# FlagArihant2000/sfm-mvs

Hardware: AMD Instinct MI355X
Metric: descriptor-pair distances/sec (BF-KNN k=2 + Lowe ratio) (higher is better)
Workload: dtype f32 results (bit-identical to the direct-form f32 reference); filter arithmetic on MFMA: i8 MFMA on the descriptors QUANTISED to 8 bits (one grid per pair; the certificate uses the measured residua...; 1 GPU; BASELINE configs[1]: 10k x 10k uniform[0,1) float32 128-D descriptors, BF-KNN k=2 + Lowe ratio 0.70; a step = one launch set = a batch of 8 distinct pairs of that shape per GPU (8e8 distances; 8 distinct pairs per launch set, 2 sets of images rotating over the steps); nq=10000, nt=10000, dim=128

## Files before the change

### sfm_mvs_amd/csrc/knn.hip

```cpp
#include "common.h"
#include <cfloat>
#include <climits>
#include <cstdlib>
#include <type_traits>
#include <algorithm>
#include <mutex>
#include <vector>

namespace {

typedef float f32x16 __attribute__((ext_vector_type(16)));
typedef float f32x4 __attribute__((ext_vector_type(4)));
typedef float f32x3 __attribute__((ext_vector_type(3), aligned(4)));
typedef int i32x3 __attribute__((ext_vector_type(3), aligned(4)));

constexpr int kDim = 128;
constexpr int kTileT = 32;


constexpr int kResidentWaves = 4096;
constexpr int kMaxSlots = 258;
constexpr float kInf = __builtin_huge_valf();
constexpr int kSubTilesHost = 64;
constexpr int kI8SubTilesHost = 128;
// ... 399 lines not shown
                    const unsigned ad = (abase ^ (32u * ((c + 2) & 7))) + ((c + 2) >= 8 ? 256u : 0u);
                    asm volatile("ds_read_b128 %0, %1" : "=v"(af[(c + 2) % 3]) : "v"(ad));
                    asm volatile("s_waitcnt lgkmcnt(2)" : "+v"(af[c % 3]));
                } else if (c + 1 < 16) {
                    asm volatile("s_waitcnt lgkmcnt(1)" : "+v"(af[c % 3]));
                } else {
                    asm volatile("s_waitcnt lgkmcnt(0)" : "+v"(af[c % 3]));
                }
                __builtin_amdgcn_sched_barrier(0);
                acc = __builtin_amdgcn_mfma_f32_32x32x2f32(af[c % 3][0], bq[4 * c + 0], acc, 0, 0, 0);
                acc = __builtin_amdgcn_mfma_f32_32x32x2f32(af[c % 3][1], bq[4 * c + 1], acc, 0, 0, 0);
                acc = __builtin_amdgcn_mfma_f32_32x32x2f32(af[c % 3][2], bq[4 * c + 2], acc, 0, 0, 0);
                acc = __builtin_amdgcn_mfma_f32_32x32x2f32(af[c % 3][3], bq[4 * c + 3], acc, 0, 0, 0);
            }
            acc = __builtin_amdgcn_mfma_f32_32x32x2f32(aug_a, aug_b, acc, 0, 0, 0);
            if (ABL & 16) __builtin_amdgcn_s_setprio(0);
            const int seq0 = (t - sub_t0) << 2;
            if (ABL & 1) {
                k0 = min(k0, __float_as_int(acc[0]) + __float_as_int(acc[15]));
            } else
#pragma unroll
            for (int r = 0; r < 16; r += 4) {
                const int key = (min(min(__float_as_int(acc[r]), __float_as_int(acc[r + 1])), min(__float_as_int(acc[r + 2]), __float_as_int(acc[r + 3]))) & ~kKeyMask) | (seq0 + (r >> 2));
                const int lo = min(key, k0), hi = max(key, k0);
                const int m1 = max(min(key, k1), min(max(key, k1), k0));
                k2 = max(min(key, k1), min(max(key, k1), k2));
                k1 = m1;
                k0 = lo;
                (void)hi;
            }
            if (!(ABL & 2)) __syncthreads();
        }

        if (qok) {
            flush_keys(k0, k1, k2, sub_t0, h, cand_s + obase + 6 * sub, cand_i + obase + 6 * sub);
            for (int e = sub + 1; e < nsub; ++e)
#pragma unroll
                for (int r = 0; r < 3; ++r) {
                    cand_s[obase + 6 * e + r] = kInf;
                    cand_i[obase + 6 * e + r] = -1;
                }
        }
        u += t_end - t_begin;
    }
    if (trace && threadIdx.x == 0) trace[4 * blockIdx.x + 1] = wall_clock64();
}

typedef __bf16 bf16x8 __attribute__((ext_vector_type(8)));
typedef _Float16 f16x8 __attribute__((ext_vector_type(8)));
typedef unsigned u32x4 __attribute__((ext_vector_type(4)));
typedef _Float16 f16x2 __attribute__((ext_vector_type(2)));
typedef float f32x2 __attribute__((ext_vector_type(2)));

__device__ __forceinline__ float dot8_f16(const uint4& a, const uint4& b, float c) {
    c = __builtin_amdgcn_fdot2(__builtin_bit_cast(f16x2, a.x), __builtin_bit_cast(f16x2, b.x), c, false);
    c = __builtin_amdgcn_fdot2(__builtin_bit_cast(f16x2, a.y), __builtin_bit_cast(f16x2, b.y), c, false);
    c = __builtin_amdgcn_fdot2(__builtin_bit_cast(f16x2, a.z), __builtin_bit_cast(f16x2, b.z), c, false);
    c = __builtin_amdgcn_fdot2(__builtin_bit_cast(f16x2, a.w), __builtin_bit_cast(f16x2, b.w), c, false);
    return c;
}

__device__ __forceinline__ unsigned bf16_rn_bits(float x) {
    const unsigned u = __float_as_uint(x);
    return (u + 0x7FFFu + ((u >> 16) & 1u)) >> 16;
}

constexpr int kModeHalfExact = 0, kModeHalf = 1, kModeSplit = 2;
constexpr int kFlagHalfInexact = 2, kFlagRangeBad = 4, kFlagNotU8 = 8, kFlagSomeU8 = 16;
constexpr int kFlagQ8 = 32;

template <int M>
__device__ __forceinline__ int lane_xor(int v) {
    if constexpr (M == 1) return __builtin_amdgcn_update_dpp(0, v, 0xB1 , 0xF, 0xF, false);
    else if constexpr (M == 2) return __builtin_amdgcn_update_dpp(0, v, 0x4E , 0xF, 0xF, false);
    else if constexpr (M == 4 || M == 8 || M == 16) return __builtin_amdgcn_ds_swizzle(v, 0x1F | (M << 10));
    else return __shfl_xor(v, M, 64);
}
template <int M>
__device__ __forceinline__ float lane_xor(float v) { return __int_as_float(lane_xor<M>(__float_as_int(v))); }
__device__ __forceinline__ int knn_filter_mode(const int* __restrict__ flags, const float* __restrict__ bmax, int lane,
                                               float* tmax_out = nullptr) {
    const int fl = flags[lane] | flags[lane + 64] | flags[lane + 128] | flags[lane + 192];
    float tmax = fmaxf(fmaxf(bmax[lane], bmax[lane + 64]), fmaxf(bmax[lane + 128], bmax[lane + 192]));
#pragma unroll
    for (int m = 32; m >= 1; m >>= 1) tmax = fmaxf(tmax, __shfl_xor(tmax, m, 64));
    if (tmax_out) *tmax_out = tmax;
    if (__any((fl & kFlagRangeBad) != 0)) return kModeSplit;
    if (!__any((fl & kFlagHalfInexact) != 0)) return kModeHalfExact;
    return tmax >= 0.25f ? kModeHalf : kModeSplit;
}

constexpr int kMinfoPairMode = 0, kMinfoBatchMode = kMaxBatch, kMinfoTmax = 16, kMinfoTerr = 24, kMinfoQmax = 32, kMinfoBase = 40, kMinfoI8 = 48,
              kMinfoQ8 = 49,
              kMinfoSub8 = 50,
              kMinfoTicket = 51,
              kMinfoQ8S = 56, kMinfoQ8Lo = 64,
              kMinfoWords = 72;
__device__ __forceinline__ int knn_batch_mode(const int* __restrict__ flags, const float* __restrict__ bmax, int n_pairs, int lane) {
    int mode = kModeHalfExact;
    for (int b = 0; b < n_pairs; ++b) mode = max(mode, knn_filter_mode(flags + b * kNormBlocks, bmax + b * kNormBlocks, lane));
    return mode;
}

constexpr int kFragBytes = 1024;
constexpr int kInitFragBytes = 512;
constexpr int kTileFragBytes = 8 * kFragBytes + kInitFragBytes;

__device__ __forceinline__ uint2 frag_init_operand(float x, bool query_side, int h) {
    unsigned hi = bf16_rn_bits(x), mid = 0, lo = 0;
    if (x < kInf) {
        const float r1 = x - __uint_as_float(hi << 16);
        mid = bf16_rn_bits(r1);
        lo = bf16_rn_bits(r1 - __uint_as_float(mid << 16));
    }
    const unsigned one = 0x3F80u;
    if (query_side) return h == 0 ? make_uint2(one | (one << 16), one | (hi << 16)) : make_uint2(mid | (lo << 16), 0u);
    return h == 0 ? make_uint2(hi | (mid << 16), lo | (one << 16)) : make_uint2(one | (one << 16), 0u);
}

constexpr int kI8Groups = 8;
constexpr int kI8Rows = 4 * kI8Groups * 32;
constexpr int kI8SubTiles = 128;
constexpr int kI8TileBytes = 5 * 1024;
constexpr int kI8QTileBytes = 4 * 1024;
constexpr int kI8CMax = 508031, kI8CMin = -503936;
static_assert(kI8SubTiles == kI8SubTilesHost, "make_plan's copy");
constexpr int kKeyEmptyI = 0x7FFFFF00;

constexpr int kQ8SubTiles = 32;
static_assert(kQ8SubTiles == kQ8SubTilesHost, "make_plan's copy");
struct Q8Grid {
    float lo, s, inv;
    int kind;
};
__device__ __forceinline__ Q8Grid q8_sample_grid(const float* __restrict__ Q, int64_t ldq, int nq, const float* __restrict__ T, int64_t ldt, int nt,
                                                 float* __restrict__ red ) {
    const int sr = threadIdx.x >> 4, c = threadIdx.x & 15;
    const float* qs = Q + (int64_t)(((int64_t)sr * nq) >> 4) * ldq + 8 * c;
    const float* ts = T + (int64_t)(((int64_t)sr * nt) >> 4) * ldt + 8 * c;
    const float4 v0 = *reinterpret_cast<const float4*>(qs), v1 = *reinterpret_cast<const float4*>(qs + 4);
    const float4 v2 = *reinterpret_cast<const float4*>(ts), v3 = *reinterpret_cast<const float4*>(ts + 4);
    const float in[16] = {v0.x, v0.y, v0.z, v0.w, v1.x, v1.y, v1.z, v1.w, v2.x, v2.y, v2.z, v2.w, v3.x, v3.y, v3.z, v3.w};
    float mn = kInf, mx = -kInf, sm = 0.f, sq = 0.f;
    bool bad = false, nonu8 = false;
#pragma unroll
    for (int e = 0; e < 16; ++e) {
        mn = fminf(mn, in[e]);
        mx = fmaxf(mx, in[e]);
        sm += in[e];
        sq = fmaf(in[e], in[e], sq);
        bad = bad || !(fabsf(in[e]) < kInf);
        nonu8 = nonu8 || !(in[e] >= 0.f && in[e] <= 255.f && in[e] == floorf(in[e]));
    }
#pragma unroll
    for (int m = 32; m >= 1; m >>= 1) {
        mn = fminf(mn, __shfl_xor(mn, m, 64));
        mx = fmaxf(mx, __shfl_xor(mx, m, 64));
        sm += __shfl_xor(sm, m, 64);
        sq += __shfl_xor(sq, m, 64);
    }
    const int fl = (__any(bad) ? 1 : 0) | (__any(nonu8) ? 2 : 0);
    __syncthreads();
    if ((threadIdx.x & 63) == 0) {
        red[5 * (threadIdx.x >> 6)] = mn;
        red[5 * (threadIdx.x >> 6) + 1] = mx;
        red[5 * (threadIdx.x >> 6) + 2] = __int_as_float(fl);
        red[5 * (threadIdx.x >> 6) + 3] = sm;
        red[5 * (threadIdx.x >> 6) + 4] = sq;
    }
    __syncthreads();
    int flw = 0;
    mn = red[0]; mx = red[1]; sm = 0.f; sq = 0.f;
#pragma unroll
    for (int w = 0; w < 4; ++w) {
        mn = fminf(mn, red[5 * w]);
        mx = fmaxf(mx, red[5 * w + 1]);
        flw |= __float_as_int(red[5 * w + 2]);
        sm += red[5 * w + 3];
        sq += red[5 * w + 4];
    }
    Q8Grid g{0.f, 1.f, 1.f, 0};
    if (flw & 1) { g.kind = 2; return g; }
    if (!(flw & 2)) return g;
    const float s = (mx - mn) * (1.f / 255.f), mabs = fmaxf(fabsf(mn), fabsf(mx));
    if (!(s >= 1e-12f && s <= 1e30f && s >= 1.52587890625e-05f * mabs)) { g.kind = 2; return g; }
    {
        const float mean = sm * (1.f / 4096.f), var = fmaxf(sq * (1.f / 4096.f) - mean * mean, 0.f);
        if (!((mx - mn) * (mx - mn) <= 25.f * var)) { g.kind = 2; return g; }
    }
    g.lo = mn; g.s = s; g.inv = 1.f / s; g.kind = 1;
    return g;
}

__device__ __forceinline__ float fp16_chunk(const float (&in)[8], float sc, unsigned (&fw)[4], unsigned& flags) {
    fw[0] = fw[1] = fw[2] = fw[3] = 0u;
    float err2 = 0.f;
    unsigned amax = 0u, umin = 0xFFFFFFFFu, dor = 0u;
#pragma unroll
    for (int e = 0; e < 8; ++e) {
        const float ev = sc * in[e];
        const _Float16 hv = (_Float16)ev;
        fw[e >> 1] |= (unsigned)__builtin_bit_cast(unsigned short, hv) << (16 * (e & 1));
        const float dv = ev - (float)hv;
        err2 = fmaf(dv, dv, err2);
        const unsigned ab = __float_as_uint(ev) & 0x7FFFFFFFu;
        amax = max(amax, ab);
        umin = min(umin, ab - 1u);
        dor |= __float_as_uint(dv);
    }
    if (amax > 0x476A6000u ) flags |= kFlagRangeBad;
    const bool has_sub = umin < 0x38800000u - 1u;
    if ((dor & 0x7FFFFFFFu) != 0u || has_sub) flags |= kFlagHalfInexact;
    if (has_sub) {
        err2 = 0.f;
#pragma unroll
        for (int e = 0; e < 8; ++e) {
            const float ev = sc * in[e];
            const float dv = fabsf(ev) < 6.103515625e-5f ? ev : ev - (float)__builtin_bit_cast(_Float16, (unsigned short)(fw[e >> 1] >> (16 * (e & 1))));
            err2 = fmaf(dv, dv, err2);
        }
    }
    return err2;
}

constexpr int kPrepThreads = 256;
__global__ __launch_bounds__(kPrepThreads) void knn_prep_kernel(BatchPtrs P, int64_t ldq, int nq, int nq_pad,
                                                       int64_t ldt, int nt, int nt_pad,
                                                       unsigned short* __restrict__ qsplit, float* __restrict__ qn,
                                                       unsigned short* __restrict__ tsplit, float* __restrict__ tn,
                                                       float* __restrict__ bmax, int* __restrict__ midflag,
                                                       float* __restrict__ qerr , float* __restrict__ bmaxerr ,
                                                       float* __restrict__ bqmax ,
                                                       int64_t s_qsplit, int64_t s_tsplit, int64_t s_qn, int64_t s_tn,
                                                       unsigned char* __restrict__ qfrag ,
                                                       unsigned char* __restrict__ tfrag, int64_t s_qfrag, int64_t s_tfrag,
                                                       int* __restrict__ zero, int nzero,
                                                       int64_t units, int tiles, int G, int seg_cost, int n_rb,
                                                       int64_t* __restrict__ wg_begin, int* __restrict__ rb_first,
                                                       int* __restrict__ rb_last, int* __restrict__ wg_sbase,
                                                       unsigned char* __restrict__ qi8, unsigned char* __restrict__ ti8, int64_t s_qi8, int64_t s_ti8,
                                                       int* __restrict__ wq , int* __restrict__ wt ,
                                                       int* __restrict__ bwmin , int* __restrict__ bwmax,
                                                       unsigned short* __restrict__ rmq ,
                                                       unsigned short* __restrict__ rmt ,
                                                       int64_t units8, int G8, int n_rb8, int64_t* __restrict__ wg_begin8,
                                                       int* __restrict__ rb_first8, int* __restrict__ rb_last8, int* __restrict__ wg_sbase8,
                                                       int q8 , int* __restrict__ minfo) {
    constexpr int kPrepWaves = kPrepThreads / 64, kPrepRows = kPrepThreads / 16;
    __shared__ float wmax[kPrepWaves];
    __shared__ float q8red[20];
    const int pb = blockIdx.y;
    if (blockIdx.x >= gridDim.x - 2) {
        if (pb == 0) {
            if (blockIdx.x == gridDim.x - 2) fill_partition_tables(make_partition(units, tiles, G, seg_cost), n_rb, wg_begin, rb_first, rb_last, wg_sbase);
            else if (qi8) {
                int sub8 = kI8SubTiles;
                if (q8)
                    for (int b = 0; b < (int)gridDim.y; ++b)
                        if (q8_sample_grid(P.q[b], ldq, nq, P.t[b], ldt, nt, q8red).kind == 1) sub8 = kQ8SubTiles;
                if (threadIdx.x == 0) { minfo[kMinfoSub8] = sub8; minfo[kMinfoTicket] = 0; }
                fill_partition_tables(make_partition(units8, tiles, G8, seg_cost), n_rb8, wg_begin8, rb_first8, rb_last8, wg_sbase8, sub8);
            }
        }
        return;
    }
    const bool do8 = qi8 != nullptr;
    if (do8) { qi8 += pb * s_qi8; ti8 += pb * s_ti8; wq += pb * s_qn; wt += pb * s_tn; bwmin += pb * kNormBlocks; bwmax += pb * kNormBlocks; rmq += pb * s_qn; rmt += pb * s_tn; }
    int w8min = INT_MAX, w8max = INT_MIN;
    const float* __restrict__ Q = P.q[pb];
    const float* __restrict__ T = P.t[pb];
    int* __restrict__ stats = P.stats[pb];
    qsplit += pb * s_qsplit; tsplit += pb * s_tsplit; qn += pb * s_qn; tn += pb * s_tn;
    bmax += pb * kNormBlocks; midflag += pb * kNormBlocks;
    qerr += pb * s_qn; bmaxerr += pb * kNormBlocks; bqmax += pb * kNormBlocks;
    zero += pb * nzero;
    const bool frag = qfrag != nullptr;
    if (frag) { qfrag += pb * s_qfrag; tfrag += pb * s_tfrag; }
    const int nblk = gridDim.x - 2;
    __shared__ int wmid[kPrepWaves];
    Q8Grid g8{0.f, 1.f, 1.f, 0};
    if (do8 && q8) g8 = q8_sample_grid(Q, ldq, nq, T, ldt, nt, q8red);
    const bool q8pair = g8.kind == 1;
    if (do8 && blockIdx.x == 0 && threadIdx.x == 0) {
        minfo[kMinfoQ8S + pb] = __float_as_int(g8.s);
        minfo[kMinfoQ8Lo + pb] = __float_as_int(g8.lo);
    }
    const int c = threadIdx.x & 15;
    float mx = 0.f, mxe = 0.f, mxq = 0.f;
    unsigned flags = 0;
    const int rows = nq_pad + nt_pad;
    constexpr int kPrepAhead = 3;
    const int row0 = blockIdx.x * kPrepRows + (threadIdx.x >> 4), rstep = nblk * kPrepRows;
    for (int rbase = row0; rbase < rows; rbase += kPrepAhead * rstep) {
    float4 vin[kPrepAhead][2];
#pragma unroll
    for (int k = 0; k < kPrepAhead; ++k) {
        const int row = rbase + k * rstep;
        const bool isq = row < nq_pad;
        const int r = isq ? row : row - nq_pad;
        vin[k][0] = vin[k][1] = make_float4(0.f, 0.f, 0.f, 0.f);
        if (row < rows && r < (isq ? nq : nt)) {
            const float* src = (isq ? Q + (int64_t)r * ldq : T + (int64_t)r * ldt) + 8 * c;
            vin[k][0] = *reinterpret_cast<const float4*>(src);
            vin[k][1] = *reinterpret_cast<const float4*>(src + 4);
        }
    }
#pragma unroll
    for (int k = 0; k < kPrepAhead; ++k) {
        const int row = rbase + k * rstep;
        if (row >= rows) break;
        const bool isq = row < nq_pad;
        const int r = isq ? row : row - nq_pad;
        const int n = isq ? nq : nt, npad = isq ? nq_pad : nt_pad;
        const float in[8] = {vin[k][0].x, vin[k][0].y, vin[k][0].z, vin[k][0].w, vin[k][1].x, vin[k][1].y, vin[k][1].z, vin[k][1].w};
        float s = ((in[0] * in[0] + in[1] * in[1]) + (in[2] * in[2] + in[3] * in[3])) + ((in[4] * in[4] + in[5] * in[5]) + (in[6] * in[6] + in[7] * in[7]));
        s += lane_xor<8>(s); s += lane_xor<4>(s); s += lane_xor<2>(s); s += lane_xor<1>(s);
        const float sc = isq ? -2.f : 1.f;
        const bool real = r < n;
        bool chunk8 = false;
        unsigned lo = 0u, hi = 0u;
        float err2q = 0.f;
        if (q8pair) {
#pragma unroll
            for (int e = 0; e < 4; ++e) {
                lo = __builtin_amdgcn_cvt_pk_u8_f32((in[e] - g8.lo) * g8.inv, e, lo);
                hi = __builtin_amdgcn_cvt_pk_u8_f32((in[4 + e] - g8.lo) * g8.inv, e, hi);
            }
            if (real) {
#pragma unroll
                for (int e = 0; e < 8; ++e) {
                    const float kf = (float)(((e < 4 ? lo : hi) >> (8 * (e & 3))) & 0xFFu);
                    const float dv = in[e] - fmaf(g8.s, kf, g8.lo);
                    err2q = fmaf(dv, dv, err2q);
                }
                flags |= kFlagQ8;
            }
            chunk8 = true;
        } else if (do8) {
            lo = __builtin_amdgcn_cvt_pk_u8_f32(in[0], 0, 0u);
            if (__any(((__float_as_uint(in[0] - (float)(lo & 0xFFu))) & 0x7FFFFFFFu) == 0u)) {
#pragma unroll
                for (int e = 0; e < 4; ++e) {
                    if (e) lo = __builtin_amdgcn_cvt_pk_u8_f32(in[e], e, lo);
                    hi = __builtin_amdgcn_cvt_pk_u8_f32(in[4 + e], e, hi);
                }
                unsigned nu = 0u;
#pragma unroll
                for (int e = 0; e < 4; ++e) {
                    nu |= __float_as_uint(in[e] - (float)((lo >> (8 * e)) & 0xFFu));
                    nu |= __float_as_uint(in[4 + e] - (float)((hi >> (8 * e)) & 0xFFu));
                }
                chunk8 = (nu & 0x7FFFFFFFu) == 0u;
            }
            if (!chunk8) flags |= kFlagNotU8;
            else if (real) flags |= kFlagSomeU8;
        }
        float err2 = 0.f;
        const float nrm = (isq || real) ? s : kInf;
        if (!__all(chunk8 && real)) {
        unsigned fw[4];
        err2 = fp16_chunk(in, sc, fw, flags);
        err2 += lane_xor<8>(err2); err2 += lane_xor<4>(err2); err2 += lane_xor<2>(err2); err2 += lane_xor<1>(err2);
        if (!(err2 < kInf)) err2 = 0.f;
        const uint4 packed = make_uint4(fw[0], fw[1], fw[2], fw[3]);
        if (frag) {
            if (!(chunk8 && real))
                *reinterpret_cast<uint4*>((isq ? qfrag : tfrag) + (int64_t)(r >> 5) * kTileFragBytes + (((c >> 1) * 64 + (c & 1) * 32 + (r & 31)) << 4)) = packed;
        } else {
            *reinterpret_cast<uint4*>((isq ? qsplit : tsplit) + (2 * (int64_t)npad + r) * kDim + 8 * c) = packed;
        }
        }
        if (q8pair) {
            err2q += lane_xor<8>(err2q); err2q += lane_xor<4>(err2q); err2q += lane_xor<2>(err2q); err2q += lane_xor<1>(err2q);
            err2 = err2q < kInf ? err2q : kInf;
        }
        if (frag && c < 2 && !isq) *reinterpret_cast<uint2*>(tfrag + (int64_t)(r >> 5) * kTileFragBytes + 8 * kFragBytes + ((c * 32 + (r & 31)) << 3)) = frag_init_operand(nrm, false, c);
        if (c == 0) (isq ? qn : tn)[r] = nrm;
        if (do8) {
            const unsigned long long m8 = __ballot(chunk8 && real);
            if (c == 0) (isq ? rmq : rmt)[r] = (unsigned short)(m8 >> (threadIdx.x & 48));
        }
        if (do8 && __any(chunk8)) {
            const unsigned flip = isq ? 0x7F7F7F7Fu : 0x80808080u;
            const unsigned x0 = real ? lo ^ flip : 0u, x1 = real ? hi ^ flip : 0u;
            int w8 = __builtin_amdgcn_sdot4((int)x0, (int)x0, 8, false);
            w8 = __builtin_amdgcn_sdot4((int)x1, (int)x1, w8, false);
            w8 = __builtin_amdgcn_sdot4((int)x0, 0x02020202, w8, false);
            w8 = __builtin_amdgcn_sdot4((int)x1, 0x02020202, w8, false);
            w8 += lane_xor<8>(w8); w8 += lane_xor<4>(w8); w8 += lane_xor<2>(w8); w8 += lane_xor<1>(w8);
            if (chunk8) {
                unsigned char* img = isq ? qi8 + (int64_t)(r >> 5) * kI8QTileBytes : ti8 + (int64_t)(r >> 5) * kI8TileBytes;
                *reinterpret_cast<uint2*>(img + (c >> 2) * 1024 + ((((c >> 1) & 1) * 32 + (r & 31)) << 4) + ((c & 1) << 3)) = make_uint2(x0, x1);
            }
            if (c == 0) (isq ? wq : wt)[r] = w8;
            if (!isq && real) { w8min = min(w8min, w8); w8max = max(w8max, w8); }
        }
        if (isq) {
            if (c == 0) qerr[r] = err2;
            mxq = fmaxf(mxq, s);
        } else {
            mx = fmaxf(mx, s);
            mxe = fmaxf(mxe, err2);
        }
    }
    }
#pragma unroll
    for (int m = 32; m >= 1; m >>= 1) {
        mx = fmaxf(mx, __shfl_xor(mx, m, 64));
        mxe = fmaxf(mxe, __shfl_xor(mxe, m, 64));
        mxq = fmaxf(mxq, __shfl_xor(mxq, m, 64));
    }
    int wfl = 0;
#pragma unroll
    for (int b = 1; b <= kFlagQ8; b <<= 1) wfl |= __any((flags & b) != 0) ? b : 0;
    __shared__ float wmaxe[kPrepWaves], wmaxq[kPrepWaves];
    __shared__ int w8lo[kPrepWaves], w8hi[kPrepWaves];
    if (do8) {
#pragma unroll
        for (int m = 32; m >= 1; m >>= 1) {
            w8min = min(w8min, __shfl_xor(w8min, m, 64));
            w8max = max(w8max, __shfl_xor(w8max, m, 64));
        }
    }
    if ((threadIdx.x & 63) == 0) {
        wmax[threadIdx.x >> 6] = mx;
        wmaxe[threadIdx.x >> 6] = mxe;
        wmaxq[threadIdx.x >> 6] = mxq;
        wmid[threadIdx.x >> 6] = wfl;
        w8lo[threadIdx.x >> 6] = w8min;
        w8hi[threadIdx.x >> 6] = w8max;
    }
    __syncthreads();
    if (threadIdx.x == 0) {
        float bm = wmax[0], bme = wmaxe[0], bmq = wmaxq[0];
        int fl = wmid[0], lo8 = w8lo[0], hi8 = w8hi[0];
        for (int w = 1; w < kPrepWaves; ++w) {
            bm = fmaxf(bm, wmax[w]);
            bme = fmaxf(bme, wmaxe[w]);
            bmq = fmaxf(bmq, wmaxq[w]);
            fl |= wmid[w];
            lo8 = min(lo8, w8lo[w]);
            hi8 = max(hi8, w8hi[w]);
        }
        bmax[blockIdx.x] = bm;
        bmaxerr[blockIdx.x] = bme;
        bqmax[blockIdx.x] = bmq;
        midflag[blockIdx.x] = fl;
        if (do8) { bwmin[blockIdx.x] = lo8; bwmax[blockIdx.x] = hi8; }
        if (blockIdx.x == 0 && stats) stats[0] = 0;
        if (blockIdx.x == 1 || nblk == 1)
            for (int i = 0; i < nzero; ++i) zero[i] = 0;
    }
}

__device__ __forceinline__ uint4 frag_init_i8(int C, int h) {
    int S = -(C >> 7);
    if (h == 1) S -= max(-15 * 128, min(15 * 127, S));
    unsigned wds[4] = {0u, 0u, 0u, 0u};
#pragma unroll
    for (int k = 0; k < 16; ++k) {
        int d;
        if (h == 0 && k == 0) d = C & 127;
        else { d = max(-128, min(127, S)); S -= d; }
        wds[k >> 2] |= (unsigned)(d & 0xFF) << (8 * (k & 3));
    }
    return make_uint4(wds[0], wds[1], wds[2], wds[3]);
}

constexpr int kSplitThreads = 512;
__global__ __launch_bounds__(kSplitThreads) void knn_split_images_kernel(BatchPtrs P, int B, int64_t ldq, int nq, int nq_pad, int64_t ldt, int nt,
                                                                        int nt_pad, unsigned short* __restrict__ qsplit0,
                                                                        unsigned short* __restrict__ tsplit0, int64_t s_qsplit, int64_t s_tsplit,
                                                                        int* __restrict__ midflag, const float* __restrict__ bmax,
                                                                        int force_mode, unsigned char* __restrict__ qhm0 ,
                                                                        unsigned char* __restrict__ thm0, int64_t s_qhm, int64_t s_thm,
                                                                        float* __restrict__ bmaxerr, const float* __restrict__ bqmax, int* __restrict__ minfo,
                                                                        unsigned char* __restrict__ ti8, int64_t s_ti8, const int* __restrict__ wt, int64_t s_tn,
                                                                        const int* __restrict__ bwmin, const int* __restrict__ bwmax,
                                                                        const unsigned char* __restrict__ qi8, int64_t s_qi8, int64_t s_qn,
                                                                        const unsigned short* __restrict__ rmq, const unsigned short* __restrict__ rmt,
                                                                        unsigned char* __restrict__ qfrag, unsigned char* __restrict__ tfrag, int64_t s_qfrag, int64_t s_tfrag,
                                                                        float* __restrict__ qerr ,
                                                                        int* __restrict__ midflag_r, float* __restrict__ bmaxerr_r ,
                                                                        int delay_wg, long long delay_ticks ) {
    if ((int)blockIdx.x == delay_wg) {
        const long long t0 = wall_clock64();
        while (wall_clock64() - t0 < delay_ticks) __builtin_amdgcn_s_sleep(8);
    }
    __shared__ int smode[kMaxBatch], s8ok[kMaxBatch], s8base[kMaxBatch], s8some[kMaxBatch], sq8[kMaxBatch];
    auto reduce_modes = [&](bool leave ) {
        const int wave = threadIdx.x >> 6, lane = threadIdx.x & 63;
        static_assert(kSplitThreads / 64 >= kMaxBatch, "one wave per pair");
        if (wave < B) {
            float tmax;
            const int m = knn_filter_mode(midflag + wave * kNormBlocks, bmax + wave * kNormBlocks, lane, &tmax);
            const float* be = bmaxerr + wave * kNormBlocks;
            const float* bq = bqmax + wave * kNormBlocks;
            float te = fmaxf(fmaxf(be[lane], be[lane + 64]), fmaxf(be[lane + 128], be[lane + 192]));
            float qm = fmaxf(fmaxf(bq[lane], bq[lane + 64]), fmaxf(bq[lane + 128], bq[lane + 192]));
#pragma unroll
            for (int sh = 32; sh >= 1; sh >>= 1) {
                te = fmaxf(te, __shfl_xor(te, sh, 64));
                qm = fmaxf(qm, __shfl_xor(qm, sh, 64));
            }
            if (ti8) {
                const int* fl = midflag + wave * kNormBlocks;
                const int* lo = bwmin + wave * kNormBlocks;
                const int* hi = bwmax + wave * kNormBlocks;
                const int fl4 = fl[lane] | fl[lane + 64] | fl[lane + 128] | fl[lane + 192];
                const bool u8 = !__any((fl4 & kFlagNotU8) != 0);
                const bool some = __any((fl4 & kFlagSomeU8) != 0);
                const bool q8p = __any((fl4 & kFlagQ8) != 0);
                int wl = min(min(lo[lane], lo[lane + 64]), min(lo[lane + 128], lo[lane + 192]));
                int wh = max(max(hi[lane], hi[lane + 64]), max(hi[lane + 128], hi[lane + 192]));
#pragma unroll
                for (int sh = 32; sh >= 1; sh >>= 1) {
                    wl = min(wl, __shfl_xor(wl, sh, 64));
                    wh = max(wh, __shfl_xor(wh, sh, 64));
                }
                const int cl = wl >> 1, ch = wh >> 1;
                const int base = max(ch - kI8CMax, min(cl + (ch - cl) / 2, cl - kI8CMin));
                const float s8 = __int_as_float(minfo[kMinfoQ8S + wave]);
                const bool fit = !q8p || (te <= 27.4f * s8 * s8 && tmax < 2.5e37f && qm < 2.5e37f);
                if (lane == 0) {
                    s8ok[wave] = (u8 && fit && wl <= wh && ch - base <= kI8CMax && cl - base >= kI8CMin) ? 1 : 0;
                    s8base[wave] = base;
                    s8some[wave] = some ? 1 : 0;
                    sq8[wave] = q8p ? 1 : 0;
                }
            }
            if (lane == 0) {
                smode[wave] = m;
                if (leave) {
                    minfo[kMinfoPairMode + wave] = m;
                    minfo[kMinfoTmax + wave] = __float_as_int(tmax);
                    minfo[kMinfoTerr + wave] = __float_as_int(te);
                    minfo[kMinfoQmax + wave] = __float_as_int(qm);
                }
            }
        }
        __syncthreads();
    };
    reduce_modes(blockIdx.x == 0);
    bool i8 = ti8 != nullptr;
    for (int b = 0; b < B && i8; ++b) i8 = s8ok[b] != 0;
    bool q8any = false, repaired = false;
    for (int b = 0; b < B && ti8; ++b) q8any = q8any || sq8[b] != 0;
    __shared__ int sq8r[kMaxBatch];
    if (threadIdx.x < kMaxBatch) sq8r[threadIdx.x] = (ti8 && q8any && !i8 && threadIdx.x < B) ? sq8[threadIdx.x] : 0;
    __syncthreads();
    if (ti8 && q8any && !i8) {
        __shared__ int rfl[kSplitThreads / 64];
        __shared__ float rme[kSplitThreads / 64];
        const int c = threadIdx.x & 15, rows = nq_pad + nt_pad;
        for (int pb = 0; pb < B; ++pb) {
            if (!sq8[pb]) continue;
            const float* __restrict__ Q = P.q[pb];
            const float* __restrict__ T = P.t[pb];
            unsigned flags = kFlagNotU8;
            float mxe = 0.f;
            if (threadIdx.x < kPrepThreads)
                for (int row = blockIdx.x * (kPrepThreads / 16) + (threadIdx.x >> 4); row < rows; row += kNormBlocks * (kPrepThreads / 16)) {
                    const bool isq = row < nq_pad;
                    const int r = isq ? row : row - nq_pad;
                    const bool real = r < (isq ? nq : nt);
                    float4 v0 = make_float4(0.f, 0.f, 0.f, 0.f), v1 = v0;
                    if (real) {
                        const float* src = (isq ? Q + (int64_t)r * ldq : T + (int64_t)r * ldt) + 8 * c;
                        v0 = *reinterpret_cast<const float4*>(src);
                        v1 = *reinterpret_cast<const float4*>(src + 4);
                    }
                    const float in[8] = {v0.x, v0.y, v0.z, v0.w, v1.x, v1.y, v1.z, v1.w};
                    unsigned fw[4];
                    float err2 = fp16_chunk(in, isq ? -2.f : 1.f, fw, flags);
                    err2 += lane_xor<8>(err2); err2 += lane_xor<4>(err2); err2 += lane_xor<2>(err2); err2 += lane_xor<1>(err2);
                    if (!(err2 < kInf)) err2 = 0.f;
                    *reinterpret_cast<uint4*>((isq ? qfrag + pb * s_qfrag : tfrag + pb * s_tfrag) + (int64_t)(r >> 5) * kTileFragBytes +
                                              (((c >> 1) * 64 + (c & 1) * 32 + (r & 31)) << 4)) = make_uint4(fw[0], fw[1], fw[2], fw[3]);
                    if (isq) { if (c == 0) qerr[pb * s_qn + r] = err2; }
                    else mxe = fmaxf(mxe, err2);
                }
            int wfl = 0;
#pragma unroll
            for (int b = 1; b <= kFlagQ8; b <<= 1) wfl |= __any((flags & b) != 0) ? b : 0;
#pragma unroll
            for (int m = 32; m >= 1; m >>= 1) mxe = fmaxf(mxe, __shfl_xor(mxe, m, 64));
            __syncthreads();
            if ((threadIdx.x & 63) == 0) { rfl[threadIdx.x >> 6] = wfl; rme[threadIdx.x >> 6] = mxe; }
            __syncthreads();
            if (threadIdx.x == 0) {
                int fl = 0;
                float me = 0.f;
                for (int w = 0; w < kPrepThreads / 64; ++w) { fl |= rfl[w]; me = fmaxf(me, rme[w]); }
                midflag_r[pb * kNormBlocks + blockIdx.x] = fl;
                bmaxerr_r[pb * kNormBlocks + blockIdx.x] = me;
            }
        }
        __shared__ int last_s;
        __builtin_amdgcn_fence(__ATOMIC_RELEASE, "agent");
        __syncthreads();
        if (threadIdx.x == 0) {
// ... 2441 lines not shown
    constexpr int kBlocks = 1024;
    SFM_CHECK_ARG(regime_max_host && trials_per_wave >= 1, "sfm_selftest_mfma_accumulation: bad argument");
    if (!ws || ws_bytes < sizeof(double) * kBlocks * 4 + 256) {
        sfm::set_error("sfm_selftest_mfma_accumulation: workspace too small (need %zu bytes)", sizeof(double) * kBlocks * 4 + 256);
        return SFM_ERR_WORKSPACE;
    }
    hipStream_t stream = sfm::as_stream(stream_);
    double* d = reinterpret_cast<double*>(sfm::align_up((size_t)(uintptr_t)ws, 256));
    static const MfmaRegime regs[7] = {
        {0, 1, 0, 1, 4, 1, 0},
        {-3, 6, -3, 6, 0, 8, 1},
        {-8, 16, -8, 16, -8, 24, 1},
        {0, 1, 0, 1, 20, 1, 1},
        {6, 2, 6, 2, -10, 4, 1},
        {-14, 4, 0, 4, -10, 8, 1},
        {-1, 2, -1, 2, 5, 3, 0},
    };
    std::vector<double> host((size_t)kBlocks * 4);
    for (int r = 0; r < 7; ++r) {
        if (use_bf16 == 2) hipLaunchKernelGGL(mfma_selftest_kernel<2>, dim3(kBlocks), dim3(256), 0, stream, regs[r], trials_per_wave, 17u + 4096u * r, d);
        else if (use_bf16) hipLaunchKernelGGL(mfma_selftest_kernel<1>, dim3(kBlocks), dim3(256), 0, stream, regs[r], trials_per_wave, 17u + 4096u * r, d);
        else hipLaunchKernelGGL(mfma_selftest_kernel<0>, dim3(kBlocks), dim3(256), 0, stream, regs[r], trials_per_wave, 17u + 4096u * r, d);
        SFM_CHECK_LAUNCH();
        SFM_CHECK_HIP(hipMemcpyAsync(host.data(), d, sizeof(double) * host.size(), hipMemcpyDeviceToHost, stream));
        SFM_CHECK_HIP(sfm::stream_sync(stream));
        double w = 0;
        for (double v : host) w = std::max(w, v);
        regime_max_host[r] = w;
    }
    return SFM_OK;
}

namespace {
struct ChainCal {
    std::once_flag once;
    float scale = -1.f;
    double worst = 0;
};
ChainCal g_chain_cal[16];
}

static float mfma_chain_scale() {
    int dev = 0;
    if (hipGetDevice(&dev) != hipSuccess || dev < 0 || dev >= 16) {
        sfm::set_error("sfm_knn2_l2_f32: no usable HIP device");
        return -1.f;
    }
    ChainCal& c = g_chain_cal[dev];
    std::call_once(c.once, [&] {
        const char* assume = getenv("SFM_KNN_ASSUME_E");
        double worst = assume && atof(assume) >= 8.0 ? atof(assume) : 0.0;
        {
            void* ws = nullptr;
            hipStream_t st = nullptr;
            if (hipMalloc(&ws, 32768 + 512) != hipSuccess || hipStreamCreateWithFlags(&st, hipStreamNonBlocking) != hipSuccess) {
                if (ws) (void)hipFree(ws);
                return;
            }
            bool ok = true;
            for (int kind = 0; kind < 3 && ok; ++kind) {
                double r[7];
                ok = sfm_selftest_mfma_accumulation(kind, 4, r, ws, 32768 + 512, st) == SFM_OK;
                for (double v : r) worst = std::max(worst, v);
            }
            (void)hipStreamDestroy(st);
            (void)hipFree(ws);
            if (!ok || !(worst < 1e6)) return;
        }
        c.worst = worst;
        c.scale = worst <= 8.0 ? 1.f : (float)(worst / 8.0);
    });
    if (c.scale < 0.f) sfm::set_error("sfm_knn2_l2_f32: the MFMA accumulation self-test could not run on device %d", dev);
    return c.scale;
}

extern "C" int sfm_knn_mfma_selftest_result(double* worst_units, float* chain_scale) {
    const float s = mfma_chain_scale();
    if (s < 0.f) return SFM_ERR_DEVICE;
    int dev = 0;
    (void)hipGetDevice(&dev);
    if (worst_units) *worst_units = g_chain_cal[dev].worst;
    if (chain_scale) *chain_scale = s;
    return SFM_OK;
}

extern "C" int sfm_debug_knn_split_delay(int workgroup, int microseconds) {
    g_split_delay_wg = workgroup;
    g_split_delay_ticks = (long long)(microseconds < 0 ? 0 : microseconds > 100000 ? 100000 : microseconds) * 100;
    return SFM_OK;
}

extern "C" int sfm_debug_set_trace(void* dev_buf) {
    g_trace = static_cast<long long*>(dev_buf);
    return SFM_OK;
}

namespace {
constexpr int64_t kMaxTrainRows = 4000000;

static_assert(kFilterHalf == 5 && kFilterNoQuant == 6, "include/sfm_hip.h SFM_KNN_FILTER_*");
bool filter_ok(int filter) { return filter >= kFilterAuto && filter <= kFilterNoQuant; }

size_t knn_ws_bytes(int64_t nq, int64_t nt, int dim, int B, int filter) {
    if (nq < 0 || nt < 0 || nt > kMaxTrainRows || dim != kDim || B < 1 || B > kMaxBatch || !filter_ok(filter)) return 0;
    if (B > 1 && filter == kFilterF32) return 0;
    const Plan p = make_plan(nq, nt, B, filter);
    if (!p.i8) return carve_ws(nullptr, nq, nt, p, nullptr).bytes + 256;
    const Plan p8 = make_plan(nq, nt, B, p.q8 ? kFilterI8PlanQ8 : kFilterI8Plan);
    return carve_ws(nullptr, nq, nt, p, &p8).bytes + 256;
}

size_t ratio_ws_bytes(int64_t nq, int B) {
    return sfm::align_up((size_t)B * (size_t)((nq + kRatioBlock - 1) / kRatioBlock * kRatioSub + 1) * sizeof(int), 256) + 256;
}

int knn_batch_impl(int B, const BatchPtrs& P, int64_t nq, int64_t ldq, int64_t nt, int64_t ldt, int dim, int filter, void* ws, size_t ws_bytes,
                   void* stream_, double ratio, int* ratio_counts, int ratio_stride) {
    SFM_CHECK_ARG(dim == kDim, "sfm_knn2_l2_f32: dim must be 128 (got %d)", dim);
    SFM_CHECK_ARG(B >= 1 && B <= kMaxBatch, "sfm_match_batch_l2_f32: 1 <= batch <= %d (got %d)", kMaxBatch, B);
    SFM_CHECK_ARG(filter_ok(filter), "sfm_knn2_l2_f32: filter must be 0 (auto), 1 (fp32 MFMA), 2 (bf16 split pinned), 3 / 4 (LDS-ring kernel, auto / split), 5 (16-bit only), 6 (auto, never quantised) (got %d)", filter);
    SFM_CHECK_ARG(nq >= 0 && nt >= 0 && nq < INT_MAX / 256 && nt <= kMaxTrainRows, "sfm_knn2_l2_f32: bad sizes nq=%lld nt=%lld (nt <= %lld)",
                  (long long)nq, (long long)nt, (long long)kMaxTrainRows);
    if (nq == 0) return SFM_OK;
    for (int b = 0; b < B; ++b) {
        SFM_CHECK_ARG(P.q[b] && P.idx[b] && P.dist[b] && (P.t[b] || nt == 0), "sfm_knn2_l2_f32: null pointer");
        SFM_CHECK_ARG(((uintptr_t)P.q[b] & 15) == 0 && ((uintptr_t)P.t[b] & 15) == 0, "sfm_knn2_l2_f32: q/t must be 16-byte aligned");
        SFM_CHECK_ARG(((uintptr_t)P.idx[b] & 7) == 0 && ((uintptr_t)P.dist[b] & 7) == 0, "sfm_knn2_l2_f32: idx/dist must be 8-byte aligned");
    }
    SFM_CHECK_ARG(ldq >= dim && ldt >= dim && ldq % 4 == 0 && ldt % 4 == 0, "sfm_knn2_l2_f32: ldq/ldt must be >= dim and multiples of 4");
    hipStream_t stream = sfm::as_stream(stream_);
    if (nt == 0) {
        for (int b = 0; b < B; ++b)
            hipLaunchKernelGGL(knn_fill_empty_kernel, dim3((unsigned)((2 * nq + 255) / 256)), dim3(256), 0, stream, P.idx[b], P.dist[b], 2 * nq, P.stats[b]);
        SFM_CHECK_LAUNCH();
        return SFM_OK;
    }
    SFM_CHECK_ARG(B == 1 || filter != kFilterF32, "sfm_match_batch_l2_f32: the fp32-MFMA filter variant is single-pair");
    const Plan p = make_plan(nq, nt, B, filter);
    Plan p8{};
    if (p.i8) p8 = make_plan(nq, nt, B, p.q8 ? kFilterI8PlanQ8 : kFilterI8Plan);
    const size_t need = knn_ws_bytes(nq, nt, dim, B, filter);
    if (!ws || ws_bytes < need) {
        sfm::set_error("sfm_knn2_l2_f32: workspace too small (%zu < %zu)", ws_bytes, need);
        return SFM_ERR_WORKSPACE;
    }
    char* base = reinterpret_cast<char*>(sfm::align_up((size_t)(uintptr_t)ws, 256));
    const KnnWs w = carve_ws(base, nq, nt, p, p.i8 ? &p8 : nullptr);
    const int nstr8 = p.i8 ? p8.smax * p8.nsub : 0;

    const dim3 grid((unsigned)p.G);
    const int prof_reps = p.split ? sfm::prof_repeat() : 1;
    static const int abl = dev_env_int("SFM_KNN_ABL", 0);
    if (p.split) {
        hipLaunchKernelGGL(knn_prep_kernel, dim3(kNormBlocks + 2, (unsigned)B), dim3(kPrepThreads), 0, stream, P, ldq, (int)nq, p.nq_pad, ldt, (int)nt,
                           p.tiles * kTileT, w.qsplit, w.qn, w.tsplit, w.tn, w.bmax, w.midflag, w.qerr, w.bmaxerr, w.bqmax, w.s_qsplit, w.s_tsplit, w.s_qn, w.s_tn,
                           p.q4 ? w.qfrag : nullptr, w.tfrag, w.s_qfrag, w.s_tfrag,
                           ratio_counts, 0 ,
                           p.units, p.tiles, p.G, p.seg_cost, p.n_rb, w.wg_begin, w.rb_first, w.rb_last, p.q4 ? w.wg_sbase : nullptr,
                           w.qi8, w.ti8, w.s_qi8, w.s_ti8, w.wq, w.wt, w.bwmin, w.bwmax, w.rmq, w.rmt, p8.units, p8.G, p8.n_rb, w.wg_begin8, w.rb_first8,
                           w.rb_last8, w.wg_sbase8, p.q8, w.minfo);
        SFM_CHECK_LAUNCH();
        hipLaunchKernelGGL(knn_split_images_kernel, dim3(kNormBlocks), dim3(kSplitThreads), 0, stream, P, B, ldq, (int)nq, p.nq_pad, ldt, (int)nt,
                           p.tiles * kTileT, w.qsplit, w.tsplit, w.s_qsplit, w.s_tsplit, w.midflag, w.bmax, p.force_mode,
                           p.q4 ? w.qhm : nullptr, w.thm, w.s_qhm, w.s_thm, w.bmaxerr, w.bqmax, w.minfo, w.ti8, w.s_ti8, w.wt, w.s_tn, w.bwmin, w.bwmax,
                           w.qi8, w.s_qi8, w.s_qn, w.rmq, w.rmt, w.qfrag, w.tfrag, w.s_qfrag, w.s_tfrag, w.qerr, w.midflag_r, w.bmaxerr_r, g_split_delay_wg, g_split_delay_ticks);
        SFM_CHECK_LAUNCH();
        sfm::prof_begin(sfm::kProfKnnFilter, stream);
#define SFM_LAUNCH_SPLIT2(A, WV)                                                                                        \
    hipLaunchKernelGGL((knn_filter_split2_kernel<A, WV>), grid, dim3(64 * WV), kRingLdsBytes + (WV == 4 ? kQScratchBytes : 0), stream, w.qsplit, w.qn,    \
                       (int)nq, p.nq_pad, w.tsplit, (int)nt, p.tiles * kTileT, w.tn, p.tiles, p.units, p.smax, p.nsub,    \
                       w.midflag, w.bmax, p.force_mode, w.cand_s, w.cand_i, w.wg_begin, w.rb_first, p.n_rb1, B, w.s_qsplit, w.s_tsplit,    \
                       w.s_qn, w.s_tn, w.s_cand, w.minfo, w.bmaxerr, g_trace)
        for (int rep = 0; rep < prof_reps; ++rep) {
        if (p.q4) {
#define SFM_LAUNCH_Q4(A)                                                                                                                         \
    hipLaunchKernelGGL(knn_filter_q4_kernel<A>, grid, dim3(256), 0, stream, w.qfrag, w.tfrag, w.qhm, w.thm, (int)nq, p.nq_pad, p.tiles, p.smax, p.nsub, \
                       w.midflag, w.bmax, p.force_mode, w.cand_s, w.cand_i, w.wg_begin, w.rb_first, p.n_rb1, B, w.s_qfrag, w.s_tfrag, w.s_qhm,         \
                       w.s_thm, w.s_cand, w.minfo, w.bmaxerr, w.wg_sbase, g_trace, w.qi8, w.ti8, w.s_qi8, w.s_ti8, w.keys8, w.sttab8, w.s_keys8, nstr8,         \
                       w.wg_begin8, p8.n_rb1, w.wg_sbase8, p8.G, (int)nt)
            if (abl == 1) SFM_LAUNCH_Q4(1); else if (abl == 2) SFM_LAUNCH_Q4(2); else if (abl == 3) SFM_LAUNCH_Q4(3); else if (abl == 4) SFM_LAUNCH_Q4(4); else SFM_LAUNCH_Q4(0);
#undef SFM_LAUNCH_Q4
        } else if (p.waves == 4) {
            if (abl == 1) SFM_LAUNCH_SPLIT2(1, 4); else if (abl == 2) SFM_LAUNCH_SPLIT2(2, 4); else if (abl == 4) SFM_LAUNCH_SPLIT2(4, 4);
            else if (abl == 6) SFM_LAUNCH_SPLIT2(6, 4); else if (abl == 7) SFM_LAUNCH_SPLIT2(7, 4); else SFM_LAUNCH_SPLIT2(0, 4);
        } else if (p.waves == 16) {
            if (abl == 1) SFM_LAUNCH_SPLIT2(1, 16); else if (abl == 7) SFM_LAUNCH_SPLIT2(7, 16); else SFM_LAUNCH_SPLIT2(0, 16);
        } else {
            if (abl == 1) SFM_LAUNCH_SPLIT2(1, 8); else if (abl == 7) SFM_LAUNCH_SPLIT2(7, 8); else SFM_LAUNCH_SPLIT2(0, 8);
        }
        }
#undef SFM_LAUNCH_SPLIT2
    } else {
    const float* q = P.q[0];
    const float* t = P.t[0];
    hipLaunchKernelGGL(knn_norms_kernel, dim3(kNormBlocks + 1), dim3(256), 0, stream, t, ldt, (int)nt, w.tn, w.bmax,
                       P.stats[0], ratio_counts, 0, p.units, p.tiles, p.G, p.seg_cost, p.n_rb, w.wg_begin, w.rb_first, w.rb_last);
    SFM_CHECK_LAUNCH();
    sfm::prof_begin(sfm::kProfKnnFilter, stream);
#define SFM_LAUNCH_FILTER(A, WV)                                                                                     \
    hipLaunchKernelGGL((knn_filter_kernel<A, WV>), grid, dim3(64 * WV), kLdsFloats * sizeof(float), stream, q, ldq,    \
                       (int)nq, t, ldt, (int)nt, w.tn, p.tiles, p.units, p.smax, p.nsub, w.cand_s, w.cand_i, g_trace)
    if (p.waves == 4) {
        switch (abl) {
            case 1: SFM_LAUNCH_FILTER(1, 4); break;
            case 7: SFM_LAUNCH_FILTER(7, 4); break;
            default: SFM_LAUNCH_FILTER(0, 4); break;
        }
    } else if (p.waves == 8) {
        switch (abl) {
            case 1: SFM_LAUNCH_FILTER(1, 8); break;
            case 7: SFM_LAUNCH_FILTER(7, 8); break;
            default: SFM_LAUNCH_FILTER(0, 8); break;
        }
    } else {
        switch (abl) {
            case 1: SFM_LAUNCH_FILTER(1, 16); break;
            case 7: SFM_LAUNCH_FILTER(7, 16); break;
            default: SFM_LAUNCH_FILTER(0, 16); break;
        }
    }
#undef SFM_LAUNCH_FILTER
    }
    sfm::prof_end(sfm::kProfKnnFilter, stream, prof_reps);
    SFM_CHECK_LAUNCH();
    const int force_mode = !p.split ? kModeF32 : p.force_mode;
    float chain_scale = 1.f;
    if (p.split) {
        chain_scale = mfma_chain_scale();
        if (chain_scale < 0.f) return SFM_ERR_DEVICE;
    }
    const int64_t refine_wgs = (int64_t)B * ((nq + kRefQ - 1) / kRefQ), refine_grid = refine_wgs >= 64 ? 8 * ((refine_wgs + 7) / 8) : refine_wgs;
    sfm::prof_begin(sfm::kProfKnnRefine, stream);
#define SFM_LAUNCH_REFINE(FRAG, THALF, S_THALF)                                                                                          \
    hipLaunchKernelGGL(knn_refine_kernel<FRAG>, dim3((unsigned)refine_grid), dim3(256), 0, stream, P, B, ldq, (int)nq, ldt, (int)nt, w.cand_s,    \
                       w.cand_i, p.rows_per_block, p.tiles, p.units, p.G, p.smax * p.nsub, p.nsub, force_mode, w.midflag, w.bmax,               \
                       p.split ? w.minfo : nullptr, p.split ? w.qerr : nullptr, w.s_qn, THALF, w.tn, w.wg_begin, w.rb_first, w.rb_last, p.n_rb1, \
                       w.s_cand, S_THALF, w.s_tn, ratio, ratio_counts, ratio_stride, chain_scale, p.q4 ? 1 : 0, g_trace ? g_trace + 16384 : nullptr,    \
                       w.qi8, w.ti8, w.s_qi8, w.s_ti8, w.wq, w.wt, w.keys8, w.sttab8, w.s_keys8, nstr8, w.rb_last8, p8.n_rb1, p8.G)
    if (p.q4) SFM_LAUNCH_REFINE(true, reinterpret_cast<const unsigned short*>(w.tfrag), w.s_tfrag / 2);
    else SFM_LAUNCH_REFINE(false, p.split ? w.tsplit + (size_t)2 * p.tiles * kTileT * kDim : nullptr, w.s_tsplit);
#undef SFM_LAUNCH_REFINE
    sfm::prof_end(sfm::kProfKnnRefine, stream);
    SFM_CHECK_LAUNCH();
    return SFM_OK;
}

BatchPtrs single_pair(const float* q, const float* t, int32_t* idx, float* dist, int32_t* stats, int32_t* out_q, int32_t* out_t,
                      int32_t* out_count, uint8_t* mask) {
    BatchPtrs P{};
    P.q[0] = q; P.t[0] = t; P.idx[0] = idx; P.dist[0] = dist; P.stats[0] = stats;
    P.out_q[0] = out_q; P.out_t[0] = out_t; P.out_count[0] = out_count; P.mask[0] = mask;
    return P;
}
}

extern "C" size_t sfm_knn2_l2_f32_ws_bytes(int64_t nq, int64_t nt, int dim, int filter) { return knn_ws_bytes(nq, nt, dim, 1, filter); }

extern "C" int sfm_knn2_l2_f32(const float* q, int64_t nq, int64_t ldq, const float* t, int64_t nt, int64_t ldt,
                               int dim, int filter, int32_t* idx, float* dist, int32_t* stats, void* ws, size_t ws_bytes,
                               void* stream_) {
    return knn_batch_impl(1, single_pair(q, t, idx, dist, stats, nullptr, nullptr, nullptr, nullptr), nq, ldq, nt, ldt, dim, filter, ws, ws_bytes,
                          stream_, 0.0, nullptr, 0);
}

extern "C" size_t sfm_ratio_compact_ws_bytes(int64_t nq) {
    if (nq < 0) return 0;
    return sfm::align_up((size_t)((nq + kRatioBlock - 1) / kRatioBlock + 1) * sizeof(int), 256) + 256;
}

extern "C" int sfm_ratio_compact(const int32_t* idx, const float* dist, int64_t nq, double ratio, int32_t* out_q,
                                 int32_t* out_t, int32_t* out_count, uint8_t* mask, void* ws, size_t ws_bytes,
                                 void* stream_) {
    SFM_CHECK_ARG(nq >= 0 && nq < INT_MAX, "sfm_ratio_compact: bad nq");
    SFM_CHECK_ARG(out_count && (nq == 0 || (idx && dist && out_q && out_t)), "sfm_ratio_compact: null pointer");
    SFM_CHECK_ARG(((uintptr_t)idx & 7) == 0 && ((uintptr_t)dist & 7) == 0, "sfm_ratio_compact: idx/dist must be 8-byte aligned");
    hipStream_t stream = sfm::as_stream(stream_);
    if (nq == 0) {
        SFM_CHECK_HIP(hipMemsetAsync(out_count, 0, sizeof(int32_t), stream));
        return SFM_OK;
    }
    if (!ws || ws_bytes < sfm_ratio_compact_ws_bytes(nq)) {
        sfm::set_error("sfm_ratio_compact: workspace too small (%zu < %zu)", ws_bytes, sfm_ratio_compact_ws_bytes(nq));
        return SFM_ERR_WORKSPACE;
    }
    int* counts = reinterpret_cast<int*>(sfm::align_up((size_t)(uintptr_t)ws, 256));
    const unsigned blocks = (unsigned)((nq + kRatioBlock - 1) / kRatioBlock);
    hipLaunchKernelGGL(ratio_count_kernel, dim3(blocks), dim3(256), 0, stream, idx, dist, (int)nq, ratio, counts, mask);
    SFM_CHECK_LAUNCH();
    hipLaunchKernelGGL(ratio_scatter_kernel, dim3(blocks), dim3(256), 0, stream, idx, dist, (int)nq, ratio, counts, out_q,
                       out_t, out_count);
    SFM_CHECK_LAUNCH();
    return SFM_OK;
}

extern "C" size_t sfm_match_batch_l2_f32_ws_bytes(int64_t nq, int64_t nt, int dim, int batch, int filter) {
    const size_t k = knn_ws_bytes(nq, nt, dim, batch, filter);
    return k ? k + ratio_ws_bytes(nq, batch) : 0;
}

extern "C" size_t sfm_match_l2_f32_ws_bytes(int64_t nq, int64_t nt, int dim, int filter) { return sfm_match_batch_l2_f32_ws_bytes(nq, nt, dim, 1, filter); }

namespace {
int match_batch_impl(int B, const BatchPtrs& P, int64_t nq, int64_t ldq, int64_t nt, int64_t ldt, int dim, int filter, double ratio, void* ws,
                     size_t ws_bytes, void* stream_) {
    SFM_CHECK_ARG(B >= 1 && B <= kMaxBatch, "sfm_match_batch_l2_f32: 1 <= batch <= %d (got %d)", kMaxBatch, B);
    SFM_CHECK_ARG(nq >= 0 && nq < INT_MAX / 256, "sfm_match_l2_f32: bad nq");
    for (int b = 0; b < B; ++b) SFM_CHECK_ARG(P.out_count[b] && (nq == 0 || (P.out_q[b] && P.out_t[b])), "sfm_match_l2_f32: null pointer");
// ... 66 lines not shown
```

Baseline: 4756 billion distances/s.

## Shrink prep grid for large batches and vectorise q8 quantisation and reductions

The prep kernel now launches fewer workgroups per pair when the batch is large (a quarter of kNormBlocks for B=8). Each workgroup writes its block statistics to several consecutive slots so downstream consumers still see kNormBlocks entries. Row indexing is made wave-uniform via readfirstlane, the q8 quantise and residual loop uses packed two-wide float math, and the shuffle reductions are unrolled into lane_xor steps with the flag bits folded into one OR-reduction. The aim is less launch and tail overhead and fewer instructions per row, at the cost of more rows per workgroup and coarser per-block bounds.

```diff
diff --git a/sfm_mvs_amd/csrc/knn.hip b/sfm_mvs_amd/csrc/knn.hip
--- a/sfm_mvs_amd/csrc/knn.hip
+++ b/sfm_mvs_amd/csrc/knn.hip
@@ -575,13 +575,12 @@
         bad = bad || !(fabsf(in[e]) < kInf);
         nonu8 = nonu8 || !(in[e] >= 0.f && in[e] <= 255.f && in[e] == floorf(in[e]));
     }
-#pragma unroll
-    for (int m = 32; m >= 1; m >>= 1) {
-        mn = fminf(mn, __shfl_xor(mn, m, 64));
-        mx = fmaxf(mx, __shfl_xor(mx, m, 64));
-        sm += __shfl_xor(sm, m, 64);
-        sq += __shfl_xor(sq, m, 64);
-    }
+    mn = fminf(mn, lane_xor<32>(mn)); mx = fmaxf(mx, lane_xor<32>(mx)); sm += lane_xor<32>(sm); sq += lane_xor<32>(sq);
+    mn = fminf(mn, lane_xor<16>(mn)); mx = fmaxf(mx, lane_xor<16>(mx)); sm += lane_xor<16>(sm); sq += lane_xor<16>(sq);
+    mn = fminf(mn, lane_xor<8>(mn)); mx = fmaxf(mx, lane_xor<8>(mx)); sm += lane_xor<8>(sm); sq += lane_xor<8>(sq);
+    mn = fminf(mn, lane_xor<4>(mn)); mx = fmaxf(mx, lane_xor<4>(mx)); sm += lane_xor<4>(sm); sq += lane_xor<4>(sq);
+    mn = fminf(mn, lane_xor<2>(mn)); mx = fmaxf(mx, lane_xor<2>(mx)); sm += lane_xor<2>(sm); sq += lane_xor<2>(sq);
+    mn = fminf(mn, lane_xor<1>(mn)); mx = fmaxf(mx, lane_xor<1>(mx)); sm += lane_xor<1>(sm); sq += lane_xor<1>(sq);
     const int fl = (__any(bad) ? 1 : 0) | (__any(nonu8) ? 2 : 0);
     __syncthreads();
     if ((threadIdx.x & 63) == 0) {
@@ -645,6 +644,9 @@
     }
     return err2;
 }
+
+__host__ __device__ constexpr int prep_blocks(int B) { return B <= 2 ? kNormBlocks : B <= 4 ? kNormBlocks / 2 : kNormBlocks / 4; }
+static_assert(kNormBlocks % prep_blocks(kMaxBatch) == 0 && kNormBlocks % prep_blocks(3) == 0, "whole words per workgroup");
 
 constexpr int kPrepThreads = 256;
 __global__ __launch_bounds__(kPrepThreads) void knn_prep_kernel(BatchPtrs P, int64_t ldq, int nq, int nq_pad,
@@ -713,16 +715,17 @@
     unsigned flags = 0;
     const int rows = nq_pad + nt_pad;
     constexpr int kPrepAhead = 3;
-    const int row0 = blockIdx.x * kPrepRows + (threadIdx.x >> 4), rstep = nblk * kPrepRows;
-    for (int rbase = row0; rbase < rows; rbase += kPrepAhead * rstep) {
+    const int lrow = (threadIdx.x >> 4) & 3;
+    const int wrow0 = __builtin_amdgcn_readfirstlane(blockIdx.x * kPrepRows + (threadIdx.x >> 4) - lrow), rstep = nblk * kPrepRows;
+    for (int wbase = wrow0; wbase < rows; wbase += kPrepAhead * rstep) {
     float4 vin[kPrepAhead][2];
 #pragma unroll
     for (int k = 0; k < kPrepAhead; ++k) {
-        const int row = rbase + k * rstep;
-        const bool isq = row < nq_pad;
-        const int r = isq ? row : row - nq_pad;
+        const int wrow = wbase + k * rstep;
+        const bool isq = wrow < nq_pad;
+        const int r = (isq ? wrow : wrow - nq_pad) + lrow;
         vin[k][0] = vin[k][1] = make_float4(0.f, 0.f, 0.f, 0.f);
-        if (row < rows && r < (isq ? nq : nt)) {
+        if (wrow < rows && r < (isq ? nq : nt)) {
             const float* src = (isq ? Q + (int64_t)r * ldq : T + (int64_t)r * ldt) + 8 * c;
             vin[k][0] = *reinterpret_cast<const float4*>(src);
             vin[k][1] = *reinterpret_cast<const float4*>(src + 4);
@@ -730,10 +733,10 @@
     }
 #pragma unroll
     for (int k = 0; k < kPrepAhead; ++k) {
-        const int row = rbase + k * rstep;
-        if (row >= rows) break;
-        const bool isq = row < nq_pad;
-        const int r = isq ? row : row - nq_pad;
+        const int wrow = wbase + k * rstep;
+        if (wrow >= rows) break;
+        const bool isq = wrow < nq_pad;
+        const int r = (isq ? wrow : wrow - nq_pad) + lrow;
         const int n = isq ? nq : nt, npad = isq ? nq_pad : nt_pad;
         const float in[8] = {vin[k][0].x, vin[k][0].y, vin[k][0].z, vin[k][0].w, vin[k][1].x, vin[k][1].y, vin[k][1].z, vin[k][1].w};
         float s = ((in[0] * in[0] + in[1] * in[1]) + (in[2] * in[2] + in[3] * in[3])) + ((in[4] * in[4] + in[5] * in[5]) + (in[6] * in[6] + in[7] * in[7]));
@@ -744,17 +747,24 @@
         unsigned lo = 0u, hi = 0u;
         float err2q = 0.f;
         if (q8pair) {
+            const f32x2 glo = {g8.lo, g8.lo}, ginv = {g8.inv, g8.inv}, gs = {g8.s, g8.s};
+            f32x2 x2[4];
+#pragma unroll
+            for (int e = 0; e < 4; ++e) x2[e] = f32x2{in[2 * e], in[2 * e + 1]};
 #pragma unroll
             for (int e = 0; e < 4; ++e) {
-                lo = __builtin_amdgcn_cvt_pk_u8_f32((in[e] - g8.lo) * g8.inv, e, lo);
-                hi = __builtin_amdgcn_cvt_pk_u8_f32((in[4 + e] - g8.lo) * g8.inv, e, hi);
+                const f32x2 u = (x2[e] - glo) * ginv;
+                if (e < 2) { lo = __builtin_amdgcn_cvt_pk_u8_f32(u.x, 2 * e, lo); lo = __builtin_amdgcn_cvt_pk_u8_f32(u.y, 2 * e + 1, lo); }
+                else { hi = __builtin_amdgcn_cvt_pk_u8_f32(u.x, 2 * e - 4, hi); hi = __builtin_amdgcn_cvt_pk_u8_f32(u.y, 2 * e - 3, hi); }
             }
             if (real) {
 #pragma unroll
-                for (int e = 0; e < 8; ++e) {
-                    const float kf = (float)(((e < 4 ? lo : hi) >> (8 * (e & 3))) & 0xFFu);
-                    const float dv = in[e] - fmaf(g8.s, kf, g8.lo);
-                    err2q = fmaf(dv, dv, err2q);
+                for (int e = 0; e < 4; ++e) {
+                    const unsigned w = e < 2 ? lo : hi;
+                    const f32x2 kf = {(float)((w >> (16 * (e & 1))) & 0xFFu), (float)((w >> (16 * (e & 1) + 8)) & 0xFFu)};
+                    const f32x2 dv = x2[e] - __builtin_elementwise_fma(gs, kf, glo);
+                    err2q = fmaf(dv.x, dv.x, err2q);
+                    err2q = fmaf(dv.y, dv.y, err2q);
                 }
                 flags |= kFlagQ8;
             }
@@ -827,24 +837,19 @@
         }
     }
     }
-#pragma unroll
-    for (int m = 32; m >= 1; m >>= 1) {
-        mx = fmaxf(mx, __shfl_xor(mx, m, 64));
-        mxe = fmaxf(mxe, __shfl_xor(mxe, m, 64));
-        mxq = fmaxf(mxq, __shfl_xor(mxq, m, 64));
-    }
-    int wfl = 0;
-#pragma unroll
-    for (int b = 1; b <= kFlagQ8; b <<= 1) wfl |= __any((flags & b) != 0) ? b : 0;
+    unsigned wflu = flags;
+    mx = fmaxf(mx, lane_xor<32>(mx)); mxe = fmaxf(mxe, lane_xor<32>(mxe)); mxq = fmaxf(mxq, lane_xor<32>(mxq));
+    wflu |= (unsigned)lane_xor<32>((int)wflu);
+    if (do8) { w8min = min(w8min, lane_xor<32>(w8min)); w8max = max(w8max, lane_xor<32>(w8max)); }
+#define SFM_PREP_TAIL_STEP(M)                                                                                              \
+    mx = fmaxf(mx, lane_xor<M>(mx)); mxe = fmaxf(mxe, lane_xor<M>(mxe)); mxq = fmaxf(mxq, lane_xor<M>(mxq));                 \
+    wflu |= (unsigned)lane_xor<M>((int)wflu);                                                                               \
+    if (do8) { w8min = min(w8min, lane_xor<M>(w8min)); w8max = max(w8max, lane_xor<M>(w8max)); }
+    SFM_PREP_TAIL_STEP(16) SFM_PREP_TAIL_STEP(8) SFM_PREP_TAIL_STEP(4) SFM_PREP_TAIL_STEP(2) SFM_PREP_TAIL_STEP(1)
+#undef SFM_PREP_TAIL_STEP
+    const int wfl = (int)(wflu & (2 * kFlagQ8 - 1));
     __shared__ float wmaxe[kPrepWaves], wmaxq[kPrepWaves];
     __shared__ int w8lo[kPrepWaves], w8hi[kPrepWaves];
-    if (do8) {
-#pragma unroll
-        for (int m = 32; m >= 1; m >>= 1) {
-            w8min = min(w8min, __shfl_xor(w8min, m, 64));
-            w8max = max(w8max, __shfl_xor(w8max, m, 64));
-        }
-    }
     if ((threadIdx.x & 63) == 0) {
         wmax[threadIdx.x >> 6] = mx;
         wmaxe[threadIdx.x >> 6] = mxe;
@@ -865,11 +870,13 @@
             lo8 = min(lo8, w8lo[w]);
             hi8 = max(hi8, w8hi[w]);
         }
-        bmax[blockIdx.x] = bm;
-        bmaxerr[blockIdx.x] = bme;
-        bqmax[blockIdx.x] = bmq;
-        midflag[blockIdx.x] = fl;
-        if (do8) { bwmin[blockIdx.x] = lo8; bwmax[blockIdx.x] = hi8; }
+        for (int j = blockIdx.x * (kNormBlocks / nblk); j < (blockIdx.x + 1) * (kNormBlocks / nblk); ++j) {
+            bmax[j] = bm;
+            bmaxerr[j] = bme;
+            bqmax[j] = bmq;
+            midflag[j] = fl;
+            if (do8) { bwmin[j] = lo8; bwmax[j] = hi8; }
+        }
         if (blockIdx.x == 0 && stats) stats[0] = 0;
         if (blockIdx.x == 1 || nblk == 1)
             for (int i = 0; i < nzero; ++i) zero[i] = 0;
@@ -3617,7 +3624,7 @@
     const int prof_reps = p.split ? sfm::prof_repeat() : 1;
     static const int abl = dev_env_int("SFM_KNN_ABL", 0);
     if (p.split) {
-        hipLaunchKernelGGL(knn_prep_kernel, dim3(kNormBlocks + 2, (unsigned)B), dim3(kPrepThreads), 0, stream, P, ldq, (int)nq, p.nq_pad, ldt, (int)nt,
+        hipLaunchKernelGGL(knn_prep_kernel, dim3(prep_blocks(B) + 2, (unsigned)B), dim3(kPrepThreads), 0, stream, P, ldq, (int)nq, p.nq_pad, ldt, (int)nt,
                            p.tiles * kTileT, w.qsplit, w.qn, w.tsplit, w.tn, w.bmax, w.midflag, w.qerr, w.bmaxerr, w.bqmax, w.s_qsplit, w.s_tsplit, w.s_qn, w.s_tn,
                            p.q4 ? w.qfrag : nullptr, w.tfrag, w.s_qfrag, w.s_tfrag,
                            ratio_counts, 0 ,
```

Result: faster. 4817 billion distances/s, median of 6 (+1.3%).
